# Polochon-street/bliss

Hardware: AMD Instinct MI355X
Metric: songs/sec bl_analyze (3-min 44.1kHz s16) + 10k x 10k distance-matrix sec (higher is better)
Workload: dtype f64; 1 GPU; configs[2] shard: 8192 synthetic 180-s 44.1 kHz s16 stereo songs/GPU resident (260.1 GB), 8192 total; step = analyze + all-gather + row-block distance; songs_per_gpu=8192, parallelism=shard1, fir_mode=2

## Files before the change

bliss_amd/csrc/bl_env_kernels.hip:

```cpp
#include <hip/hip_runtime.h>
#include <atomic>
#include <algorithm>
#include <stdlib.h>

#include "bl_launch.h"
#include "bl_fft_tan.h"
#include "bl_metric.h"
#include "bl_fir.h"
#include "bl_tail.h"

#define EV_CWAVES 7
#define EV_TILE (4 * EV_CWAVES)
#define EV_TROW 258

template <int CTRL> __device__ __forceinline__ double bl_dpp_f64(double v) {
  const unsigned long long b = __double_as_longlong(v);
  const int lo = __builtin_amdgcn_update_dpp(0, (int)(unsigned)(b & 0xFFFFFFFFull), CTRL, 0xF, 0xF, true);
  const int hi = __builtin_amdgcn_update_dpp(0, (int)(unsigned)(b >> 32), CTRL, 0xF, 0xF, true);
  return __longlong_as_double(((unsigned long long)(unsigned)hi << 32) | (unsigned)lo);
}

template <int CTRL> __device__ __forceinline__ double bl_dpp_f64_old(double old, double v) {
  const unsigned long long b = __double_as_longlong(v), o = __double_as_longlong(old);
  const int lo = __builtin_amdgcn_update_dpp((int)(unsigned)(o & 0xFFFFFFFFull), (int)(unsigned)(b & 0xFFFFFFFFull),
// ... 69 lines not shown
  const int n_units = EV_CWAVES * (int)gridDim.x;
  auto run_begin = [&](int u) -> int { return (int)((long long)n_rounds * u / n_units); };
  const int u0 = EV_CWAVES * (int)blockIdx.x;
  int steps = 0;
  for (int c = 0; c < EV_CWAVES; ++c) steps = max(steps, run_begin(u0 + c + 1) - run_begin(u0 + c));
  const int n_used = 256 * (sg.n_windows + 1);
  int seq = 0;

  if (wave == EV_CWAVES) {
    __builtin_amdgcn_s_setprio(3);
    {
      const int rowi = min(ln & 31, EV_TILE - 1);
      const bool own = ln < 32;
      const int c2 = min(rowi >> 2, EV_CWAVES - 1);
      const int q0 = run_begin(u0 + c2), q1 = run_begin(u0 + c2 + 1);
      const double2 *row = reinterpret_cast<const double2 *>(terms + rowi * EV_TROW);
      const double2 *zero2 = reinterpret_cast<const double2 *>(smem + EV3_ZERO_OFF);
      const double2 *tp = own ? row : row + 65;
      const double2 *tail = own ? row + 64 : zero2;
      float psum = 0.f;
      for (int st = 1; st <= steps + 1; ++st) {
        stamp(st - 1, 0);
        for (;;) {
          const int f = ln < EV_CWAVES ? flags[ln] : st;
          if (__all(f >= st)) break;
          __builtin_amdgcn_s_sleep(1);
        }
        ev_lds_acquire();
        stamp(st - 1, 1);
        const int rr = own ? st : st - 1;
        const int rho = q0 + rr - 1, w = 4 * rho + (ln & 3);
        const bool live = (ln & 31) < EV_TILE && rr >= 1 && rr <= steps && rho < q1 && w < sg.n_windows;
        const float carried = __shfl(psum, ln & 31);
        float sum = own ? 0.f : carried;
        if (live) {
          double2 ta[8], tb2[8];
#define EV_LOAD8(T, B) _Pragma("unroll") for (int k = 0; k < 8; ++k) T[k] = tp[8 * (B) + k];
#define EV_SUM8(T)                                                                                      \
  _Pragma("unroll") for (int k = 0; k < 8; ++k) {                                                       \
    sum = (float)((double)sum + T[k].x);                                                                \
    sum = (float)((double)sum + T[k].y);                                                                \
  }
#define EV_SB __builtin_amdgcn_sched_barrier(0);
          EV_LOAD8(ta, 0) EV_LOAD8(tb2, 1) EV_SB
          EV_SUM8(ta) EV_SB EV_LOAD8(ta, 2) EV_SB
          EV_SUM8(tb2) EV_SB EV_LOAD8(tb2, 3) EV_SB
          EV_SUM8(ta) EV_SB EV_LOAD8(ta, 4) EV_SB
          EV_SUM8(tb2) EV_SB EV_LOAD8(tb2, 5) EV_SB
          EV_SUM8(ta) EV_SB EV_LOAD8(ta, 6) EV_SB
          EV_SUM8(tb2) EV_SB EV_LOAD8(tb2, 7)
          const double2 tl = tail[0];
          EV_SB
          EV_SUM8(ta) EV_SB
          EV_SUM8(tb2)
          sum = (float)((double)sum + tl.x);
          sum = (float)((double)sum + tl.y);
#undef EV_LOAD8
#undef EV_SUM8
#undef EV_SB
        }
        ev_lds_release();
        if (ln == 0) flags[8] = st;
        psum = sum;
        if (live && !own) {
          energies[sg.env_off + w] = sum;
          lc[sg.env_off + w] = bl_tail_compress((double)sum, tb.log101);
        }
        stamp(st - 1, 2);
      }
    }
    return;
  }

  auto phase = [&](int k) {
    const int pr = (PRIO >> (4 * k)) & 3;
    if (pr == 0) __builtin_amdgcn_s_setprio(0);
    else if (pr == 1) __builtin_amdgcn_s_setprio(1);
    else if (pr == 2) __builtin_amdgcn_s_setprio(2);
    else __builtin_amdgcn_s_setprio(3);
  };
  double *buf = reinterpret_cast<double *>(smem) + wave * EV3_SLOTS;
  const int mean = st.mean;
  const double rcp = st.rcp, rcp_lo = st.rcp_lo;
#define FC(m) st.firc[m]
  auto nrm = [&](int k) -> double { return FIR_MODE == 2 ? (double)k : bl_norm(k, rcp, rcp_lo); };
  const int r0 = run_begin(u0 + wave), r1 = run_begin(u0 + wave + 1);
  constexpr bool EV3_TAN = FIR_MODE != 0;
  double t1[16];
  bl_fft16_fold<double> fold;
  c2d w1r[16];
  if (EV3_TAN) {
    const bl_fft_tan_lane<double> *tl = reinterpret_cast<const bl_fft_tan_lane<double> *>(tb.tan_lane) + l;
    t1[0] = 0.0;
#pragma unroll
    for (int k1 = 1; k1 < 16; ++k1) {
      t1[k1] = tl->t1[k1];
      asm volatile("" : "+v"(t1[k1]));
    }
    fold = tl->fold;
#define EV3_PIN(A, N) _Pragma("unroll") for (int i = 0; i < N; ++i) asm volatile("" : "+v"(A[i]));
    EV3_PIN(fold.rb, 4) EV3_PIN(fold.rc, 4) EV3_PIN(fold.rd, 4) EV3_PIN(fold.fb, 4) EV3_PIN(fold.fc, 2) EV3_PIN(fold.g, 3)
#undef EV3_PIN
  } else {
#pragma unroll
    for (int k1 = 1; k1 < 16; ++k1) {
      w1r[k1] = tw256[k1 * 16 + l];
      asm volatile("" : "+v"(w1r[k1].re), "+v"(w1r[k1].im));
    }
  }
  int base5 = (4 * r0) % 5;

  if (r0 < r1) {
    const int s0 = 1024 * r0 + 4 * ln;
    double r[20];
#pragma unroll
    for (int u = 0; u < 5; ++u) {
      const int i0 = s0 - 16 + 4 * u;
      const bool ok = i0 >= 0 && i0 + 4 <= n_used;
      const uint2 v = *reinterpret_cast<const uint2 *>(p + (ok ? i0 : 0));
      const unsigned w[2] = {ok ? v.x : 0u, ok ? v.y : 0u};
#pragma unroll
      for (int k = 0; k < 2; ++k) {
        const int lo = (int)(short)(w[k] & 0xFFFFu), hi = (int)(short)(w[k] >> 16);
        r[4 * u + 2 * k] = ok ? nrm(lo - mean) : 0.0;
        r[4 * u + 2 * k + 1] = ok ? nrm(hi - mean) : 0.0;
      }
    }
    double *dst = buf + base5 * EV3_BLK + EV3_ROW(ln >> 2) + EV3_UNIT(2 * (ln & 3));
#pragma unroll
    for (int i = 0; i < 4; ++i) {
#define XW(m) r[i + 16 - (m)]
      dst[EV3_UNIT(i >> 1) + (i & 1)] = BL_FIR_SEL(FIR_MODE, XW, FC);
#undef XW
    }
  }

  uint4 pre[4];
  short preh;
#if defined(__HIP_DEVICE_COMPILE__) && !defined(__gfx950__)
#error "k_env_windows3: the raw-buffer descriptor and its range check are written for gfx950"
#endif
  const __amdgpu_buffer_rsrc_t prs =
      __builtin_amdgcn_make_buffer_rsrc(const_cast<int16_t *>(p), 0, (int)(2u * (unsigned)n_used), 0x00020000);
  unsigned voff = 2u * (unsigned)(1024 * r0 + 240 + 16 * ln);
  unsigned voffh = 2u * (unsigned)(1024 * r0 + 256 * g + l);
  typedef unsigned ev_v4u __attribute__((__vector_size__(16)));
  auto fetch = [&]() {
#pragma unroll
    for (int u = 0; u < 4; ++u) {
      const ev_v4u v = __builtin_amdgcn_raw_buffer_load_b128(prs, (int)(voff + 16u * u), 0, 0);
      pre[u] = make_uint4(v[0], v[1], v[2], v[3]);
    }
    preh = (short)__builtin_amdgcn_raw_buffer_load_b16(prs, (int)voffh, 0, 0);
    voff += 2048u;
    voffh += 2048u;
  };
  fetch();
  double held[8];
#pragma unroll
  for (int k0 = 0; k0 < 8; ++k0) held[k0] = 0.0;
  auto publish_held_only = [&]() {
    while (__builtin_amdgcn_readfirstlane(flags[8]) < seq - 1) __builtin_amdgcn_s_sleep(1);
    ev_lds_acquire();
    double *tg = terms + (4 * wave + g) * EV_TROW;
#pragma unroll
    for (int k0 = 0; k0 < 8; ++k0)
      if (k0 < 7 || l != 15) tg[256 - l - 16 * k0] = held[k0];
    ev_wave_sync();
  };
  for (int s = 0; s < steps; ++s) {
    ++seq;
    const int rho = r0 + s;
    if (rho >= r1) {
      publish_held_only();
      if (ln == 0) flags[wave] = seq;
      continue;
    }
    stamp(s, 0);
    phase(0);
    double yv[16], yh;
    {
      double r[32];
#pragma unroll
      for (int u = 0; u < 4; ++u) {
        const unsigned w[4] = {pre[u].x, pre[u].y, pre[u].z, pre[u].w};
#pragma unroll
        for (int k = 0; k < 4; ++k) {
          const int lo = (int)(short)(w[k] & 0xFFFFu), hi = (int)(short)(w[k] >> 16);
          r[8 * u + 2 * k] = nrm(lo - mean);
          r[8 * u + 2 * k + 1] = nrm(hi - mean);
        }
      }
      const int kh = (int)preh - mean;
      const double xh = nrm(kh);
      fetch();
#pragma unroll
      for (int i = 0; i < 16; ++i) {
#define XR(m) r[i + 16 - (m)]
        yv[i] = BL_FIR_SEL(FIR_MODE, XR, FC);
#undef XR
      }
      if (FIR_MODE == 2) {
#define KH(m) __builtin_amdgcn_update_dpp(0, kh, 0x110 + (m), 0xF, 0xF, true)
        const double p0 = (double)kh;
        const double p1 = (double)(KH(1) + KH(15)), p2 = (double)(KH(2) + KH(14)), p3 = (double)(KH(3) + KH(13));
        const double p4 = (double)(KH(4) + KH(12)), p5 = (double)(KH(5) + KH(11)), p6 = (double)(KH(6) + KH(10));
        const double p7 = (double)(KH(7) + KH(9)), p8 = (double)KH(8);
#undef KH
        double y_ = FC(7) * p7;
        y_ = __builtin_fma(FC(6), p6, y_);
        y_ = __builtin_fma(FC(5), p5, y_);
        y_ = __builtin_fma(FC(4), p4, y_);
        y_ = __builtin_fma(FC(3), p3, y_);
        y_ = __builtin_fma(FC(2), p2, y_);
        y_ = __builtin_fma(FC(1), p1, y_);
        y_ = __builtin_fma(p8, FC(8), y_);
        yh = __builtin_fma(FC(0), p0, y_);
      } else {
      double hx[17];
      hx[0] = xh;
      hx[1] = bl_dpp_f64<0x111>(xh);  hx[2] = bl_dpp_f64<0x112>(xh);  hx[3] = bl_dpp_f64<0x113>(xh);
      hx[4] = bl_dpp_f64<0x114>(xh);  hx[5] = bl_dpp_f64<0x115>(xh);  hx[6] = bl_dpp_f64<0x116>(xh);
      hx[7] = bl_dpp_f64<0x117>(xh);  hx[8] = bl_dpp_f64<0x118>(xh);  hx[9] = bl_dpp_f64<0x119>(xh);
      hx[10] = bl_dpp_f64<0x11A>(xh); hx[11] = bl_dpp_f64<0x11B>(xh); hx[12] = bl_dpp_f64<0x11C>(xh);
      hx[13] = bl_dpp_f64<0x11D>(xh); hx[14] = bl_dpp_f64<0x11E>(xh); hx[15] = bl_dpp_f64<0x11F>(xh);
      hx[16] = 0.0;
#define XH(m) hx[m]
      yh = BL_FIR_SEL(FIR_MODE, XH, FC);
#undef XH
      }
    }
    const int xa = base5 + g, xb = xa + 1;
    const int pa = xa >= 5 ? xa - 5 : xa, pb = xb >= 5 ? xb - 5 : xb;
    double *blk_a = buf + pa * EV3_BLK, *blk_b = buf + pb * EV3_BLK;
    stamp(s, 1);
    phase(1);
    ev_wave_sync();
#pragma unroll
    for (int i = 0; i < 16; ++i) blk_b[EV3_ROW(l) + EV3_UNIT(i >> 1) + (i & 1)] = yv[i];
    buf[EV3_HEADS + ln] = yh;
    ev_wave_sync();
    double re[16], im[16];
    {
      const int off = EV3_ROW(l >> 3) + EV3_UNIT(l & 7);
      const double *ia = blk_a + off, *ib = blk_b + off;
      const double *i0 = l < 8 ? buf + EV3_HEADS + 16 * g + 2 * l : ia;
      re[0] = i0[0];
      im[0] = i0[1];
#pragma unroll
      for (int m1 = 1; m1 < 8; ++m1) { re[m1] = ia[EV3_ROW(2 * m1)]; im[m1] = ia[EV3_ROW(2 * m1) + 1]; }
#pragma unroll
      for (int m1 = 8; m1 < 16; ++m1) { re[m1] = ib[EV3_ROW(2 * (m1 - 8))]; im[m1] = ib[EV3_ROW(2 * (m1 - 8)) + 1]; }
    }
    ev_wave_sync();
    stamp(s, 2);
    phase(2);
    if (EV3_TAN) {
      bl_fft512_pass1_tan(re, im, t1);
    } else {
      bl_fft16(re, im);
#pragma unroll
      for (int k1 = 1; k1 < 16; ++k1) bl_cmul(re[bl_pos16(k1)], im[bl_pos16(k1)], w1r[k1].re, w1r[k1].im);
    }
    stamp(s, 3);
    phase(3);
    double *xg = blk_a;
    const double2 *xrow = reinterpret_cast<const double2 *>(xg + l * 18);
#pragma unroll
    for (int k1 = 0; k1 < 16; ++k1) xg[k1 * 18 + l] = re[bl_pos16(k1)];
    ev_wave_sync();
#pragma unroll
    for (int q = 0; q < 8; ++q) { const double2 v = xrow[q]; re[2 * q] = v.x; re[2 * q + 1] = v.y; }
    ev_wave_sync();
#pragma unroll
    for (int k1 = 0; k1 < 16; ++k1) xg[k1 * 18 + l] = im[bl_pos16(k1)];
    ev_wave_sync();
#pragma unroll
    for (int q = 0; q < 8; ++q) { const double2 v = xrow[q]; im[2 * q] = v.x; im[2 * q + 1] = v.y; }
    ev_wave_sync();
    stamp(s, 4);
    phase(4);
    double *tg = terms + (4 * wave + g) * EV_TROW;
    stamp(s, 5);
    phase(5);
    while (__builtin_amdgcn_readfirstlane(flags[8]) < seq - 1) {}
    ev_lds_acquire();
    stamp(s, 6);
#pragma unroll
    for (int k0 = 0; k0 < 8; ++k0)
      if (k0 < 7 || l != 15) tg[256 - l - 16 * k0] = held[k0];
    if (EV3_TAN) bl_fft16_folded(re, im, fold);
    else bl_fft16(re, im);
    double mir7 = 0.0;
#pragma unroll
    for (int k0 = 0; k0 < 8; ++k0) {
      const double sr = re[bl_pos16(15 - k0)], si = im[bl_pos16(15 - k0)];
      const double zr = k0 ? re[bl_pos16(16 - k0)] : re[bl_pos16(0)];
      const double zi = k0 ? im[bl_pos16(16 - k0)] : im[bl_pos16(0)];
      const double pr = bl_dpp_f64_old<0x111>(zr, bl_dpp_f64<0x140>(sr));
      const double pi = bl_dpp_f64_old<0x111>(zi, bl_dpp_f64<0x140>(si));
      double own;
      if (EV3_TAN)
        bl_fft512_power1_tan<double, false>(re[bl_pos16(k0)], im[bl_pos16(k0)], pr, pi, tw512[l + 16 * k0], own, held[k0]);
      else
        bl_fft512_power1<double, false>(re[bl_pos16(k0)], im[bl_pos16(k0)], pr, pi, tw512[l + 16 * k0], own, held[k0]);
      tg[l + 16 * k0] = own;
      if (k0 == 7) mir7 = held[7];
    }
    const double mr = re[bl_pos16(8)], mi = im[bl_pos16(8)];
    const double mid = 4.0 * __builtin_fma(mr, mr, mi * mi);
    if (l == 0) tg[128] = mid;
    if (l == 15) tg[129] = mir7;
    ev_wave_sync();
    if (ln == 0) flags[wave] = seq;
    stamp(s, 7);
    base5 = base5 == 0 ? 4 : base5 - 1;
  }
  ++seq;
  publish_held_only();
  if (ln == 0) flags[wave] = seq;
}
#undef FC

#define BL_TAIL_OMAX 48

__global__ __launch_bounds__(192) void k_env_tail(const bl_dsong *__restrict__ songs,
                                                  const double *__restrict__ lc, int n_songs,
                                                  bl_amd_song_result *res, int what) {
  __shared__ double yblk[2][38 * 64];
  __shared__ double oblk[2][BL_TAIL_OMAX * 64];
  __shared__ int ocnt[2][64];
  __shared__ double rings_ab[29 * 64];
  __shared__ double rings_c[19 * 64];
  __shared__ int flag_mem[4];
  typedef __attribute__((address_space(3))) volatile int lds_vint;
  lds_vint *flags = (lds_vint *)flag_mem;
  __builtin_amdgcn_s_setprio(3);
  const int wave = __builtin_amdgcn_readfirstlane(threadIdx.x >> 6), lane = threadIdx.x & 63;
  const int song = blockIdx.x * 64 + lane;
  const bool valid = song < n_songs;
  bl_dsong sg;
  if (valid) sg = songs[song];
  else { sg.nb_frames = 0; sg.n_windows = 0; sg.env_off = 0; sg.n = 1; sg.duration = 1; }
  const int N = 2 * sg.nb_frames;
  int maxN = N;
#pragma unroll
  for (int off = 32; off > 0; off >>= 1) maxN = max(maxN, __shfl_xor(maxN, off));
  if (threadIdx.x < 4) flags[threadIdx.x] = 0;
  __syncthreads();
  const int n_blocks = (maxN + 37) / 38;

  if (wave == 0) {
    bl_tail_iir a;
    a.init();
    const double *mylc = lc + sg.env_off;
    const int nw = sg.n_windows;
    auto fetch = [&](int kb_, double (&dst)[19]) {
#pragma unroll
      for (int q = 0; q < 19; ++q) dst[q] = mylc[max(min(19 * kb_ + q, nw - 1), 0)];
    };
    auto block = [&](int kb, double (&cur)[19], double (&fut)[19]) {
      if (kb >= n_blocks) return;
      fetch(kb + 2, fut);
      double *yo = yblk[kb & 1] + lane;
      double ye[38];
#pragma unroll
      for (int q = 0; q < 19; ++q) a.pair(19 * kb + q < nw ? cur[q] : 0.0, ye[2 * q], ye[2 * q + 1]);
      while (__builtin_amdgcn_readfirstlane(flags[1]) < kb - 1) __builtin_amdgcn_s_sleep(1);
      ev_lds_acquire();
#pragma unroll
      for (int q = 0; q < 38; ++q) yo[q * 64] = ye[q];
      ev_lds_release();
      bl_wave_sync();
      if (lane == 0) flags[0] = kb + 1;
    };
    double pa[19], pb[19], pc[19];
    fetch(0, pa);
    fetch(1, pb);
    for (int kb = 0; kb < n_blocks; kb += 3) {
      block(kb, pa, pc);
      block(kb + 1, pb, pa);
      block(kb + 2, pc, pb);
    }
    return;
  }

  if (wave == 1) {
    bl_tail_ab t;
    t.init(sg.nb_frames, rings_ab + lane, 64);
    for (int kb = 0; kb < n_blocks; ++kb) {
      while (__builtin_amdgcn_readfirstlane(flags[0]) < kb + 1) __builtin_amdgcn_s_sleep(1);
      while (__builtin_amdgcn_readfirstlane(flags[3]) < kb - 1) __builtin_amdgcn_s_sleep(1);
      ev_lds_acquire();
      const double *yin = yblk[kb & 1] + lane;
      const int j = 38 * kb;
      bl_tail_fifo f;
      f.base = oblk[kb & 1] + lane;
      f.stride = 64;
      f.count = 0;
      if (bl_tail_ab::chunk_ok(j, N)) {
        t.fast_chunk38(yin, 64, f.base, 64);
        f.count = 38;
      } else if (j < N) {
        for (int q = 0; q < 38; ++q) {
          const int jj = j + q;
// ... 117 lines not shown
```

bliss_amd/csrc/bl_fir.h:

```cpp
#ifndef BL_FIR_H_
#define BL_FIR_H_

#include <hip/hip_runtime.h>

#define BL_C0 (-0.0023470)
#define BL_C1 0.0044613
#define BL_C2 (-0.0114627)
#define BL_C3 0.0226382
#define BL_C4 (-0.0405147)
#define BL_C5 0.0580037
#define BL_C6 (-0.0779167)
#define BL_C7 0.0882711
#define BL_C8 0.9065095

__device__ __forceinline__ double bl_norm(int k, double rcp, double rcp_lo) {
  const double kd = (double)k;
  return __builtin_fma(kd, rcp, kd * rcp_lo);
}

#define BL_FIR(X)                                                   \
  ({                                                                \
    double y_ = BL_C7 * (X(7) + X(9));                              \
    y_ += BL_C6 * (X(6) + X(10));                                   \
    y_ += BL_C5 * (X(5) + X(11));                                   \
    y_ += BL_C4 * (X(4) + X(12));                                   \
    y_ += BL_C3 * (X(3) + X(13));                                   \
    y_ += BL_C2 * (X(2) + X(14));                                   \
    y_ += BL_C1 * (X(1) + X(15));                                   \
    y_ += X(8) * BL_C8;                                             \
    y_ += BL_C0 * (X(0) + X(16));                                   \
    y_;                                                             \
  })

#define BL_FIR_FUSED(X)                                             \
  ({                                                                \
    double y_ = BL_C7 * (X(7) + X(9));                              \
    y_ = __builtin_fma(BL_C6, X(6) + X(10), y_);                    \
    y_ = __builtin_fma(BL_C5, X(5) + X(11), y_);                    \
    y_ = __builtin_fma(BL_C4, X(4) + X(12), y_);                    \
    y_ = __builtin_fma(BL_C3, X(3) + X(13), y_);                    \
    y_ = __builtin_fma(BL_C2, X(2) + X(14), y_);                    \
    y_ = __builtin_fma(BL_C1, X(1) + X(15), y_);                    \
    y_ = __builtin_fma(X(8), BL_C8, y_);                            \
    y_ = __builtin_fma(BL_C0, X(0) + X(16), y_);                    \
    y_;                                                             \
  })
#define BL_FIR_FOLD(X, FC)                                          \
  ({                                                                \
    double y_ = FC(7) * (X(7) + X(9));                              \
    y_ = __builtin_fma(FC(6), X(6) + X(10), y_);                    \
    y_ = __builtin_fma(FC(5), X(5) + X(11), y_);                    \
    y_ = __builtin_fma(FC(4), X(4) + X(12), y_);                    \
    y_ = __builtin_fma(FC(3), X(3) + X(13), y_);                    \
    y_ = __builtin_fma(FC(2), X(2) + X(14), y_);                    \
    y_ = __builtin_fma(FC(1), X(1) + X(15), y_);                    \
    y_ = __builtin_fma(X(8), FC(8), y_);                            \
    y_ = __builtin_fma(FC(0), X(0) + X(16), y_);                    \
    y_;                                                             \
  })
#ifndef BL_FIR_FUSED_DEFAULT
#define BL_FIR_FUSED_DEFAULT 2
#endif
#define BL_FIR_SEL(MODE, X, FC) ((MODE) == 2 ? BL_FIR_FOLD(X, FC) : (MODE) == 1 ? BL_FIR_FUSED(X) : BL_FIR(X))

#endif
```

bliss_amd/csrc/bl_launch.h:

```cpp
#ifndef BL_LAUNCH_H_
#define BL_LAUNCH_H_

#include <hip/hip_runtime.h>
#include <stddef.h>
#include <stdint.h>
#include <stdio.h>

#include "bl_device.h"
#include "bl_fft.h"

#define BL_HIP_CHECK(expr)                                                              \
  do {                                                                                  \
    hipError_t e_ = (expr);                                                             \
    if (e_ != hipSuccess) {                                                             \
      fprintf(stderr, "bliss_amd: %s failed: %s (%s:%d)\n", #expr, hipGetErrorString(e_), \
              __FILE__, __LINE__);                                                      \
      return BL_UNEXPECTED;                                                             \
    }                                                                                   \
  } while (0)


struct bl_dsong {
  unsigned long long pcm_off;
  unsigned long long duration;
  long long env_off;
  int n, channels;
  int n_frames;
  int nb_frames;
  int n_windows;
  int reserved0;
  int out_idx;
  int reserved1;
};

struct bl_dstats {
  unsigned long long sum;
  unsigned long long sumsq;
  unsigned first;
  int last;
  int mean, variance;
  double vprime;
  double rcp;
  double rcp_lo;
  int wrap_pass;
  int status;
  long long wrap_acc;
  double firc[9];
};

typedef bl_c2<double> c2d;
typedef bl_c2<float> c2f;

struct bl_tables {
  const c2d *tw256_d, *tw512_d;
  const float *hann;
  const c2f *lv_tw;
  float lv_leafc[4];
  const double *tan_lane;
  const c2d *tw512t;
  double log101;
};


enum { PK_SCAN, PK_AMP, PK_FREQ, PK_FREQ_FIN, PK_ENV, PK_TAIL, PK_DIST, PK_FREQ_SCAN, PK_COUNT };

typedef void (*blk_mark_fn)(void *user, int kernel_id, hipStream_t stream, int begin);

struct Mark {
  blk_mark_fn fn;
  void *user;
  int k;
  hipStream_t s;
  Mark(blk_mark_fn f, void *u, int kk, hipStream_t ss) : fn(f), user(u), k(kk), s(ss) {
    if (fn) fn(user, k, s, 1);
  }
  ~Mark() {
    if (fn) fn(user, k, s, 0);
  }
};

inline int grid_x_for(long long units_max, int n_songs, int blocks_per_cu, int n_cu) {
  long long want = ((long long)n_cu * blocks_per_cu + n_songs - 1) / n_songs;
  if (want < 1) want = 1;
  if (want > units_max) want = units_max;
  if (want < 1) want = 1;
  if (want > 65535) want = 65535;
  return (int)want;
}


size_t blk_tables_bytes(void);
void blk_tables_fill_host(unsigned char *h);
bl_tables blk_tables_bind(const void *d_mem);
int blk_configure_device(void);

struct blk_analyze_args {
  const int16_t *pcm;
  const bl_dsong *songs;
  bl_dstats *stats;
  unsigned *hist;
  float *spectrum;
  float *energies;
  double *lc;
  bl_amd_song_result *results;
  int n_songs, max_n, what, n_cu;
  int n_head = 0, max_n_rest = 0;
  bl_tables tb;
  hipStream_t stream, side;
  hipEvent_t ev_env, ev_tail;
  hipStream_t side2 = nullptr;
  hipEvent_t ev_head = nullptr, ev_tail2 = nullptr;
  blk_mark_fn mark;
  void *mark_user;
};
int blk_analyze(const blk_analyze_args &a);


void blk_stats_init(const blk_analyze_args &a);
int blk_pcm_scan(const blk_analyze_args &a);
void blk_song_prep(const blk_analyze_args &a);
void blk_amp_finish(const blk_analyze_args &a, hipStream_t s);
void blk_force(const blk_analyze_args &a);
int blk_freq_configure_device(void);
bool blk_freq_scan_fused(int what);
void blk_freq_scan(const blk_analyze_args &a);
void blk_freq_frames(const blk_analyze_args &a, hipStream_t s);
void blk_freq_finish(const blk_analyze_args &a, hipStream_t s);
int blk_env_configure_device(void);
int blk_fir_mode();
int blk_env_windows(const blk_analyze_args &a, int fir_mode, int first, int count, int maxn);
// ... 92 lines not shown
```

bliss_amd/csrc/bl_stats_kernels.hip:

```cpp
#include <hip/hip_runtime.h>
#include <math.h>

#include "bl_launch.h"
#include "bl_scan.h"
#include "bl_fir.h"


template <bool HIST>
__global__ __launch_bounds__(256) void k_pcm_scan(const int16_t *__restrict__ pcm,
                                                  const bl_dsong *__restrict__ songs,
                                                  bl_dstats *stats, unsigned *hist) {
  __shared__ unsigned lh[BL_HIST_BINS];
  if (__builtin_amdgcn_groupstaticsize() != sizeof lh) __builtin_trap();
  const int tid = threadIdx.x;
  const bl_dsong sg = songs[blockIdx.y];
  const int16_t *p = pcm + sg.pcm_off;
  for (int i = tid; i < BL_HIST_BINS; i += 256) lh[i] = 0;
  __syncthreads();
  unsigned lds_base = (unsigned)(size_t)(bl_lds_u32 *)lh;
  asm volatile("" : "+v"(lds_base));

  long long sum = 0;
  unsigned long long sq = 0;
  const unsigned nvec = (unsigned)sg.n >> 3;
// ... 29 lines not shown
  if ((tid & 63) == 0) {
    atomicAdd(&st->sum, (unsigned long long)sum);
    atomicAdd(&st->sumsq, sq);
  }
  asm volatile("s_waitcnt lgkmcnt(0)" ::: "memory");
  __syncthreads();
  unsigned *gh = hist + (size_t)blockIdx.y * BL_HIST_BINS;
  for (int i = tid; i < BL_HIST_BINS; i += 256) {
    const unsigned c = lh[i];
    if (c) atomicAdd(&gh[i], c);
  }
}

__global__ __launch_bounds__(128) void k_trim(const int16_t *__restrict__ pcm, const bl_dsong *__restrict__ songs,
                                              bl_dstats *stats) {
  const bl_dsong sg = songs[blockIdx.x];
  const int16_t *p = pcm + sg.pcm_off;
  const uint4 *pv = reinterpret_cast<const uint4 *>(p);
  const int lane = threadIdx.x & 63, n = sg.n;
  const int nvec = n >> 3;
  const bool fwd = __builtin_amdgcn_readfirstlane(threadIdx.x >> 6) == 0;
  bl_dstats *st = stats + blockIdx.x;
  auto locate = [&](const uint4 q) -> int {
    const unsigned w[4] = {q.x, q.y, q.z, q.w};
    int at = fwd ? 8 : -1;
#pragma unroll
    for (int k = 0; k < 4; ++k) {
      if (fwd) {
        if (w[3 - k] >> 16) at = 2 * (3 - k) + 1;
        if (w[3 - k] & 0xFFFFu) at = 2 * (3 - k);
      } else {
        if (w[k] & 0xFFFFu) at = 2 * k;
        if (w[k] >> 16) at = 2 * k + 1;
      }
    }
    return at;
  };
  if (fwd) {
    unsigned first = 0xFFFFFFFFu;
    for (int v0 = 0; v0 < nvec; v0 += 128) {
      const int va = v0 + lane, vb = v0 + 64 + lane;
      const uint4 z = make_uint4(0, 0, 0, 0);
      const uint4 qa = va < nvec ? pv[va] : z, qb = vb < nvec ? pv[vb] : z;
      const unsigned long long ma = __ballot((qa.x | qa.y | qa.z | qa.w) != 0u);
      const unsigned long long mb = __ballot((qb.x | qb.y | qb.z | qb.w) != 0u);
      if (ma | mb) {
        const int src = ma ? __builtin_ctzll(ma) : __builtin_ctzll(mb);
        const unsigned mine = 8u * (unsigned)(ma ? va : vb) + (unsigned)locate(ma ? qa : qb);
        first = (unsigned)__shfl((int)mine, src);
        break;
      }
    }
    if (first == 0xFFFFFFFFu)
      for (int i = 8 * nvec; i < n; ++i)
        if (p[i] != 0) { first = (unsigned)i; break; }
    if (lane == 0) st->first = first;
  } else {
    int last = -1;
    for (int i = n - 1; i >= 8 * nvec; --i)
      if (p[i] != 0) { last = i; break; }
    if (last < 0)
      for (int v1 = nvec; v1 > 0; v1 -= 128) {
        const int va = v1 - 1 - lane, vb = v1 - 65 - lane;
        const uint4 z = make_uint4(0, 0, 0, 0);
        const uint4 qa = va >= 0 ? pv[va] : z, qb = vb >= 0 ? pv[vb] : z;
        const unsigned long long ma = __ballot((qa.x | qa.y | qa.z | qa.w) != 0u);
        const unsigned long long mb = __ballot((qb.x | qb.y | qb.z | qb.w) != 0u);
        if (ma | mb) {
          const int src = ma ? __builtin_ctzll(ma) : __builtin_ctzll(mb);
          const int mine = 8 * (ma ? va : vb) + locate(ma ? qa : qb);
          last = __shfl(mine, src);
          break;
        }
      }
    if (lane == 0) st->last = last;
  }
}

__global__ void k_stats_init(bl_dstats *stats, int n_songs) {
  const int i = blockIdx.x * blockDim.x + threadIdx.x;
  if (i >= n_songs) return;
  bl_dstats s;
  s.sum = 0; s.sumsq = 0; s.first = 0xFFFFFFFFu; s.last = -1;
  s.mean = 0; s.variance = 0; s.vprime = 0; s.rcp = 0; s.rcp_lo = 0; s.wrap_pass = 0; s.status = BL_OK;
  s.wrap_acc = 0;
  stats[i] = s;
}


__device__ __forceinline__ void prep_finish(bl_dstats &s, int n) {
  if (s.variance == 0) s.status = BL_UNEXPECTED;
  s.vprime = (double)s.variance / 32768.0;
  const double v2 = 2.0 * s.vprime;
  s.rcp = 1.0 / v2;
  s.rcp_lo = __builtin_fma(-s.rcp, v2, 1.0) / v2;
  const double taps[9] = {BL_C0, BL_C1, BL_C2, BL_C3, BL_C4, BL_C5, BL_C6, BL_C7, BL_C8};
#pragma unroll
  for (int m = 0; m < 9; ++m) s.firc[m] = __builtin_fma(taps[m], s.rcp, taps[m] * s.rcp_lo);
  (void)n;
}

__global__ void k_song_prep(const bl_dsong *__restrict__ songs, bl_dstats *stats, int n_songs,
                            bl_amd_song_result *res) {
  const int i = blockIdx.x * blockDim.x + threadIdx.x;
  if (i >= n_songs) return;
  bl_dstats s = stats[i];
  const bl_dsong sg = songs[i];
  const int n = sg.n;
  if (s.first == 0xFFFFFFFFu) {
    s.status = BL_UNEXPECTED;
    s.first = 0; s.last = n - 1;
  }
  const int wrapped = (int)(unsigned)(s.sum & 0xFFFFFFFFull);
  s.mean = wrapped / n;
  const long long m = s.mean;
  if (m > 13571 || m < -13571) {
    s.wrap_pass = 1;
  } else {
    const long long acc = (long long)s.sumsq - 2 * m * (long long)s.sum + (long long)n * m * m;
    s.variance = (int)(acc / n);
    prep_finish(s, n);
  }
  stats[i] = s;
  bl_amd_song_result *r = res + sg.out_idx;
  r->start = (int)s.first; r->end = s.last;
  r->mean = s.mean; r->variance = s.variance;
  r->n_frames = sg.n_frames; r->nb_frames = sg.nb_frames; r->n_windows = sg.n_windows;
  r->status = s.status;
}

__global__ __launch_bounds__(256) void k_variance_wrap(const int16_t *__restrict__ pcm,
                                                       const bl_dsong *__restrict__ songs,
                                                       bl_dstats *stats) {
  bl_dstats *st = stats + blockIdx.y;
  if (!st->wrap_pass) return;
  const bl_dsong sg = songs[blockIdx.y];
  const int16_t *p = pcm + sg.pcm_off;
  const int mean = st->mean;
  long long acc = 0;
  for (unsigned i = blockIdx.x * 256u + threadIdx.x; i < (unsigned)sg.n; i += gridDim.x * 256u) {
    const int v = (int)p[i] - mean;
    acc += (int)((unsigned)v * (unsigned)v);
  }
#pragma unroll
  for (int off = 32; off > 0; off >>= 1) acc += __shfl_down(acc, off);
  if ((threadIdx.x & 63) == 0)
    atomicAdd(reinterpret_cast<unsigned long long *>(&st->wrap_acc), (unsigned long long)acc);
}

__global__ void k_variance_wrap_finish(const bl_dsong *__restrict__ songs, bl_dstats *stats,
                                       int n_songs, bl_amd_song_result *res) {
  const int i = blockIdx.x * blockDim.x + threadIdx.x;
  if (i >= n_songs) return;
  bl_dstats s = stats[i];
  if (!s.wrap_pass) return;
  s.variance = (int)(s.wrap_acc / songs[i].n);
  prep_finish(s, songs[i].n);
  stats[i] = s;
  res[songs[i].out_idx].variance = s.variance;
  res[songs[i].out_idx].status = s.status;
}


#define BL_AMP_PASSES 301
#define BL_INT_LO ((32767 - 1000) - BL_HIST_LO)
#define BL_INT_HI ((32767 + 1000) - BL_HIST_LO)

__global__ __launch_bounds__(256) void k_amp_finish(const bl_dsong *__restrict__ songs,
                                                    const bl_dstats *__restrict__ stats,
                                                    const unsigned *__restrict__ hist,
                                                    bl_amd_song_result *res) {
  __shared__ float buf[2][BL_HIST_BINS + 8];
  const int tid = threadIdx.x;
  const int song = blockIdx.x;
  const bl_dstats st = stats[song];
  const int n = songs[song].n;
  const unsigned *gh = hist + (size_t)song * BL_HIST_BINS;
  const int start = (int)st.first, end = st.last;
  if (tid < 8) {
    const int c = tid < 3 ? tid : BL_HIST_BINS + tid;
    buf[0][c] = 0.f; buf[1][c] = 0.f;
// ... 111 lines not shown
```

Before: 23970 songs/s.

## Compute FIR filter with int8 MFMA on byte-split samples and integer taps

In FIR mode 2, the 17-tap symmetric FIR over raw integer PCM samples now runs on int8 matrix instructions. The integer-scaled taps are split into signed byte planes and the samples into low and high byte planes. The partial products are recombined exactly in int32 and then scaled once by a per-song factor, replacing the per-song scaled f64 tap array with a single scale. The sample fetch layout is changed to feed the MFMA operands, and the filtered outputs are scattered to the LDS ring in a new pattern. This removes many f64 FMAs per sample, at the cost of extra MFMA issue, byte permutes and a possible change in rounding from tap quantization.

```diff
diff --git a/bliss_amd/csrc/bl_env_kernels.hip b/bliss_amd/csrc/bl_env_kernels.hip
--- a/bliss_amd/csrc/bl_env_kernels.hip
+++ b/bliss_amd/csrc/bl_env_kernels.hip
@@ -175,7 +175,7 @@
   double *buf = reinterpret_cast<double *>(smem) + wave * EV3_SLOTS;
   const int mean = st.mean;
   const double rcp = st.rcp, rcp_lo = st.rcp_lo;
-#define FC(m) st.firc[m]
+  const double fsc = st.fsc;
   auto nrm = [&](int k) -> double { return FIR_MODE == 2 ? (double)k : bl_norm(k, rcp, rcp_lo); };
   const int r0 = run_begin(u0 + wave), r1 = run_begin(u0 + wave + 1);
   constexpr bool EV3_TAN = FIR_MODE != 0;
@@ -201,6 +201,19 @@
       asm volatile("" : "+v"(w1r[k1].re), "+v"(w1r[k1].im));
     }
   }
+  typedef int ev_v4i __attribute__((ext_vector_type(4)));
+  unsigned cp[4][2];
+  ev_v4i ini0, ini2, ini4;
+  if (FIR_MODE == 2) {
+    bl_firi_tap_planes(l, g, cp);
+#pragma unroll
+    for (int j = 0; j < 4; ++j) asm volatile("" : "+v"(cp[j][0]), "+v"(cp[j][1]));
+    int k0, k2, k4;
+    bl_firi_const(mean, &k0, &k2, &k4);
+    ini0 = ev_v4i{k0, k0, k0, k0};
+    ini2 = ev_v4i{k2, k2, k2, k2};
+    ini4 = ev_v4i{k4, k4, k4, k4};
+  }
   int base5 = (4 * r0) % 5;
 
   if (r0 < r1) {
@@ -223,7 +236,7 @@
 #pragma unroll
     for (int i = 0; i < 4; ++i) {
 #define XW(m) r[i + 16 - (m)]
-      dst[EV3_UNIT(i >> 1) + (i & 1)] = BL_FIR_SEL(FIR_MODE, XW, FC);
+      dst[EV3_UNIT(i >> 1) + (i & 1)] = BL_FIR_SEL(FIR_MODE, XW, fsc);
 #undef XW
     }
   }
@@ -235,13 +248,13 @@
 #endif
   const __amdgpu_buffer_rsrc_t prs =
       __builtin_amdgcn_make_buffer_rsrc(const_cast<int16_t *>(p), 0, (int)(2u * (unsigned)n_used), 0x00020000);
-  unsigned voff = 2u * (unsigned)(1024 * r0 + 240 + 16 * ln);
+  unsigned voff = 2u * (unsigned)(1024 * r0 + 240 + (FIR_MODE == 2 ? 16 * l + 8 * g : 16 * ln));
   unsigned voffh = 2u * (unsigned)(1024 * r0 + 256 * g + l);
   typedef unsigned ev_v4u __attribute__((__vector_size__(16)));
   auto fetch = [&]() {
 #pragma unroll
     for (int u = 0; u < 4; ++u) {
-      const ev_v4u v = __builtin_amdgcn_raw_buffer_load_b128(prs, (int)(voff + 16u * u), 0, 0);
+      const ev_v4u v = __builtin_amdgcn_raw_buffer_load_b128(prs, (int)(voff + (FIR_MODE == 2 ? 512u : 16u) * u), 0, 0);
       pre[u] = make_uint4(v[0], v[1], v[2], v[3]);
     }
     preh = (short)__builtin_amdgcn_raw_buffer_load_b16(prs, (int)voffh, 0, 0);
@@ -272,7 +285,42 @@
     stamp(s, 0);
     phase(0);
     double yv[16], yh;
-    {
+    const int kh = (int)preh - mean;
+    if (FIR_MODE == 2) {
+      ev_v4i acc[4][5];
+#pragma unroll
+      for (int t = 0; t < 4; ++t) {
+        const unsigned w[4] = {pre[t].x, pre[t].y, pre[t].z, pre[t].w};
+        unsigned lp[2], hp[2];
+        bl_firi_sample_planes(w, lp, hp);
+        const ev_v4i smp = {(int)lp[0], (int)lp[1], (int)hp[0], (int)hp[1]};
+        const ev_v4i zero = {0, 0, 0, 0};
+#define EV3_W64(A, B) (long)(((unsigned long long)(B) << 32) | (unsigned long long)(A))
+#define EV3_TAP2(J) ev_v4i{(int)cp[(J) + 1][0], (int)cp[(J) + 1][1], (int)cp[J][0], (int)cp[J][1]}
+        acc[t][0] = __builtin_amdgcn_mfma_i32_16x16x32_i8(EV3_W64(cp[0][0], cp[0][1]), EV3_W64(lp[0], lp[1]), ini0, 0, 0, 0);
+        acc[t][1] = __builtin_amdgcn_mfma_i32_16x16x64_i8(EV3_TAP2(0), smp, zero, 0, 0, 0);
+        acc[t][2] = __builtin_amdgcn_mfma_i32_16x16x64_i8(EV3_TAP2(1), smp, ini2, 0, 0, 0);
+        acc[t][3] = __builtin_amdgcn_mfma_i32_16x16x64_i8(EV3_TAP2(2), smp, zero, 0, 0, 0);
+        acc[t][4] = __builtin_amdgcn_mfma_i32_16x16x32_i8(EV3_W64(cp[3][0], cp[3][1]), EV3_W64(hp[0], hp[1]), ini4, 0, 0, 0);
+#undef EV3_W64
+#undef EV3_TAP2
+      }
+      fetch();
+#pragma unroll
+      for (int t = 0; t < 4; ++t)
+#pragma unroll
+        for (int r = 0; r < 4; ++r)
+          yv[4 * t + r] = bl_firi_combine(acc[t][0][r], acc[t][1][r], acc[t][2][r], acc[t][3][r], acc[t][4][r]) * fsc;
+#define KH(m) __builtin_amdgcn_update_dpp(0, kh, 0x110 + (m), 0xF, 0xF, true)
+      const double hp_[9] = {(double)kh ,
+                             (double)(KH(1) + KH(15)), (double)(KH(2) + KH(14)), (double)(KH(3) + KH(13)),
+                             (double)(KH(4) + KH(12)), (double)(KH(5) + KH(11)), (double)(KH(6) + KH(10)),
+                             (double)(KH(7) + KH(9)), (double)KH(8)};
+#undef KH
+#define XP(m) hp_[m]
+      yh = BL_FIR_INT_P(XP) * fsc;
+#undef XP
+    } else {
       double r[32];
 #pragma unroll
       for (int u = 0; u < 4; ++u) {
@@ -284,32 +332,14 @@
           r[8 * u + 2 * k + 1] = nrm(hi - mean);
         }
       }
-      const int kh = (int)preh - mean;
       const double xh = nrm(kh);
       fetch();
 #pragma unroll
       for (int i = 0; i < 16; ++i) {
 #define XR(m) r[i + 16 - (m)]
-        yv[i] = BL_FIR_SEL(FIR_MODE, XR, FC);
+        yv[i] = BL_FIR_SEL(FIR_MODE, XR, fsc);
 #undef XR
       }
-      if (FIR_MODE == 2) {
-#define KH(m) __builtin_amdgcn_update_dpp(0, kh, 0x110 + (m), 0xF, 0xF, true)
-        const double p0 = (double)kh;
-        const double p1 = (double)(KH(1) + KH(15)), p2 = (double)(KH(2) + KH(14)), p3 = (double)(KH(3) + KH(13));
-        const double p4 = (double)(KH(4) + KH(12)), p5 = (double)(KH(5) + KH(11)), p6 = (double)(KH(6) + KH(10));
-        const double p7 = (double)(KH(7) + KH(9)), p8 = (double)KH(8);
-#undef KH
-        double y_ = FC(7) * p7;
-        y_ = __builtin_fma(FC(6), p6, y_);
-        y_ = __builtin_fma(FC(5), p5, y_);
-        y_ = __builtin_fma(FC(4), p4, y_);
-        y_ = __builtin_fma(FC(3), p3, y_);
-        y_ = __builtin_fma(FC(2), p2, y_);
-        y_ = __builtin_fma(FC(1), p1, y_);
-        y_ = __builtin_fma(p8, FC(8), y_);
-        yh = __builtin_fma(FC(0), p0, y_);
-      } else {
       double hx[17];
       hx[0] = xh;
       hx[1] = bl_dpp_f64<0x111>(xh);  hx[2] = bl_dpp_f64<0x112>(xh);  hx[3] = bl_dpp_f64<0x113>(xh);
@@ -319,9 +349,8 @@
       hx[13] = bl_dpp_f64<0x11D>(xh); hx[14] = bl_dpp_f64<0x11E>(xh); hx[15] = bl_dpp_f64<0x11F>(xh);
       hx[16] = 0.0;
 #define XH(m) hx[m]
-      yh = BL_FIR_SEL(FIR_MODE, XH, FC);
+      yh = BL_FIR_SEL(FIR_MODE, XH, fsc);
 #undef XH
-      }
     }
     const int xa = base5 + g, xb = xa + 1;
     const int pa = xa >= 5 ? xa - 5 : xa, pb = xb >= 5 ? xb - 5 : xb;
@@ -329,8 +358,18 @@
     stamp(s, 1);
     phase(1);
     ev_wave_sync();
-#pragma unroll
-    for (int i = 0; i < 16; ++i) blk_b[EV3_ROW(l) + EV3_UNIT(i >> 1) + (i & 1)] = yv[i];
+    if (FIR_MODE == 2) {
+#pragma unroll
+      for (int t = 0; t < 4; ++t) {
+        const int xt = base5 + t + 1, pt = xt >= 5 ? xt - 5 : xt;
+        double *d = buf + pt * EV3_BLK + EV3_ROW(l) + EV3_UNIT(2 * g);
+#pragma unroll
+        for (int r = 0; r < 4; ++r) d[EV3_UNIT(r >> 1) + (r & 1)] = yv[4 * t + r];
+      }
+    } else {
+#pragma unroll
+      for (int i = 0; i < 16; ++i) blk_b[EV3_ROW(l) + EV3_UNIT(i >> 1) + (i & 1)] = yv[i];
+    }
     buf[EV3_HEADS + ln] = yh;
     ev_wave_sync();
     double re[16], im[16];
@@ -413,7 +452,6 @@
   publish_held_only();
   if (ln == 0) flags[wave] = seq;
 }
-#undef FC
 
 #define BL_TAIL_OMAX 48
 
diff --git a/bliss_amd/csrc/bl_fir.h b/bliss_amd/csrc/bl_fir.h
--- a/bliss_amd/csrc/bl_fir.h
+++ b/bliss_amd/csrc/bl_fir.h
@@ -2,6 +2,7 @@
 #define BL_FIR_H_
 
 #include <hip/hip_runtime.h>
+#include "bl_fir_int.h"
 
 #define BL_C0 (-0.0023470)
 #define BL_C1 0.0044613
@@ -45,22 +46,9 @@
     y_ = __builtin_fma(BL_C0, X(0) + X(16), y_);                    \
     y_;                                                             \
   })
-#define BL_FIR_FOLD(X, FC)                                          \
-  ({                                                                \
-    double y_ = FC(7) * (X(7) + X(9));                              \
-    y_ = __builtin_fma(FC(6), X(6) + X(10), y_);                    \
-    y_ = __builtin_fma(FC(5), X(5) + X(11), y_);                    \
-    y_ = __builtin_fma(FC(4), X(4) + X(12), y_);                    \
-    y_ = __builtin_fma(FC(3), X(3) + X(13), y_);                    \
-    y_ = __builtin_fma(FC(2), X(2) + X(14), y_);                    \
-    y_ = __builtin_fma(FC(1), X(1) + X(15), y_);                    \
-    y_ = __builtin_fma(X(8), FC(8), y_);                            \
-    y_ = __builtin_fma(FC(0), X(0) + X(16), y_);                    \
-    y_;                                                             \
-  })
 #ifndef BL_FIR_FUSED_DEFAULT
 #define BL_FIR_FUSED_DEFAULT 2
 #endif
-#define BL_FIR_SEL(MODE, X, FC) ((MODE) == 2 ? BL_FIR_FOLD(X, FC) : (MODE) == 1 ? BL_FIR_FUSED(X) : BL_FIR(X))
+#define BL_FIR_SEL(MODE, X, SC) ((MODE) == 2 ? BL_FIR_INT(X) * (SC) : (MODE) == 1 ? BL_FIR_FUSED(X) : BL_FIR(X))
 
 #endif
diff --git a/bliss_amd/csrc/bl_fir_int.h b/bliss_amd/csrc/bl_fir_int.h
--- /dev/null
+++ b/bliss_amd/csrc/bl_fir_int.h
@@ -0,0 +1,118 @@
+#ifndef BL_FIR_INT_H_
+#define BL_FIR_INT_H_
+
+#if defined(__HIPCC__)
+#include <hip/hip_runtime.h>
+#define BL_FIRI_HD __host__ __device__ __forceinline__
+#else
+#include <math.h>
+#define BL_FIRI_HD static inline
+#endif
+
+#define BL_CI0 (-23470.0)
+#define BL_CI1 44613.0
+#define BL_CI2 (-114627.0)
+#define BL_CI3 226382.0
+#define BL_CI4 (-405147.0)
+#define BL_CI5 580037.0
+#define BL_CI6 (-779167.0)
+#define BL_CI7 882711.0
+#define BL_CI8 9065095.0
+#define BL_FIRI_TAPSUM 9887759LL
+#define BL_FIRI_UNSCALE 1e7
+
+BL_FIRI_HD int bl_firi_tap(int m) {
+  if (m < 0 || m > 16) return 0;
+  switch (m > 8 ? 16 - m : m) {
+    case 0: return (int)BL_CI0;
+    case 1: return (int)BL_CI1;
+    case 2: return (int)BL_CI2;
+    case 3: return (int)BL_CI3;
+    case 4: return (int)BL_CI4;
+    case 5: return (int)BL_CI5;
+    case 6: return (int)BL_CI6;
+    case 7: return (int)BL_CI7;
+    default: return (int)BL_CI8;
+  }
+}
+
+BL_FIRI_HD int bl_firi_digit(int c, int j) {
+  for (int i = 0; i < j; ++i) c = (c - (int)(signed char)(c & 255)) / 256;
+  return (int)(signed char)(c & 255);
+}
+
+#define BL_FIR_INT_P(P)                                             \
+  ({                                                                \
+    double y_ = BL_CI7 * P(7);                                      \
+    y_ = __builtin_fma(BL_CI6, P(6), y_);                           \
+    y_ = __builtin_fma(BL_CI5, P(5), y_);                           \
+    y_ = __builtin_fma(BL_CI4, P(4), y_);                           \
+    y_ = __builtin_fma(BL_CI3, P(3), y_);                           \
+    y_ = __builtin_fma(BL_CI2, P(2), y_);                           \
+    y_ = __builtin_fma(BL_CI1, P(1), y_);                           \
+    y_ = __builtin_fma(P(8), BL_CI8, y_);                           \
+    y_ = __builtin_fma(BL_CI0, P(0), y_);                           \
+    y_;                                                             \
+  })
+#define BL_FIR_INT_PAIR_(X, m) ((m) == 8 ? X(8) : X(m) + X(16 - (m)))
+#define BL_FIR_INT(X)                                               \
+  ({                                                                \
+    const double ps_[9] = {BL_FIR_INT_PAIR_(X, 0), BL_FIR_INT_PAIR_(X, 1), BL_FIR_INT_PAIR_(X, 2),  \
+                           BL_FIR_INT_PAIR_(X, 3), BL_FIR_INT_PAIR_(X, 4), BL_FIR_INT_PAIR_(X, 5),  \
+                           BL_FIR_INT_PAIR_(X, 6), BL_FIR_INT_PAIR_(X, 7), BL_FIR_INT_PAIR_(X, 8)}; \
+    BL_FIR_INT_P(BL_FIR_INT_PS_);                                   \
+  })
+#define BL_FIR_INT_PS_(m) ps_[m]
+
+BL_FIRI_HD double bl_firi_scale(double rcp, double rcp_lo) {
+  const double q = rcp / BL_FIRI_UNSCALE;
+  const double r = __builtin_fma(-q, BL_FIRI_UNSCALE, rcp) + rcp_lo;
+  return q + r / BL_FIRI_UNSCALE;
+}
+
+
+BL_FIRI_HD int bl_firi_kappa(int kb, int q, int e) { return 8 * kb + 4 * q + e; }
+
+BL_FIRI_HD unsigned bl_firi_perm(unsigned hi, unsigned lo, unsigned sel) {
+#if defined(__HIP_DEVICE_COMPILE__)
+  return __builtin_amdgcn_perm(hi, lo, sel);
+#else
+  const unsigned long long v = ((unsigned long long)hi << 32) | lo;
+  unsigned r = 0;
+  for (int i = 0; i < 4; ++i) r |= (unsigned)((v >> (8 * ((sel >> (8 * i)) & 7))) & 255) << (8 * i);
+  return r;
+#endif
+}
+
+BL_FIRI_HD void bl_firi_sample_planes(const unsigned w[4], unsigned lp[2], unsigned hp[2]) {
+  for (int q = 0; q < 2; ++q) {
+    lp[q] = bl_firi_perm(w[2 * q + 1], w[2 * q], 0x06040200u) ^ 0x80808080u;
+    hp[q] = bl_firi_perm(w[2 * q + 1], w[2 * q], 0x07050301u);
+  }
+}
+
+BL_FIRI_HD void bl_firi_tap_planes(int b, int kb, unsigned cp[4][2]) {
+  for (int q = 0; q < 2; ++q) {
+    unsigned v[4] = {0, 0, 0, 0};
+    for (int e = 0; e < 4; ++e) {
+      const int c = bl_firi_tap(16 + b - bl_firi_kappa(kb, q, e));
+      for (int j = 0; j < 4; ++j) v[j] |= (unsigned)(bl_firi_digit(c, j) & 255) << (8 * e);
+    }
+    for (int j = 0; j < 4; ++j) cp[j][q] = v[j];
+  }
+}
+
+BL_FIRI_HD void bl_firi_const(int mean, int *k0, int *k2, int *k4) {
+  const long long K = (long long)(128 - mean) * BL_FIRI_TAPSUM;
+  *k0 = (int)(K & 0xFFFF);
+  *k2 = (int)((K >> 16) & 0xFFFF);
+  *k4 = (int)(K >> 32);
+}
+
+BL_FIRI_HD double bl_firi_combine(int a0, int a1, int a2, int a3, int a4) {
+  const int lo = a0 + a1 * 256;
+  const int mid = a2 + a3 * 256 + a4 * 65536;
+  return __builtin_fma((double)mid, 65536.0, (double)lo);
+}
+
+#endif
diff --git a/bliss_amd/csrc/bl_launch.h b/bliss_amd/csrc/bl_launch.h
--- a/bliss_amd/csrc/bl_launch.h
+++ b/bliss_amd/csrc/bl_launch.h
@@ -45,7 +45,7 @@
   int wrap_pass;
   int status;
   long long wrap_acc;
-  double firc[9];
+  double fsc;
 };
 
 typedef bl_c2<double> c2d;
diff --git a/bliss_amd/csrc/bl_stats_kernels.hip b/bliss_amd/csrc/bl_stats_kernels.hip
--- a/bliss_amd/csrc/bl_stats_kernels.hip
+++ b/bliss_amd/csrc/bl_stats_kernels.hip
@@ -135,7 +135,7 @@
   if (i >= n_songs) return;
   bl_dstats s;
   s.sum = 0; s.sumsq = 0; s.first = 0xFFFFFFFFu; s.last = -1;
-  s.mean = 0; s.variance = 0; s.vprime = 0; s.rcp = 0; s.rcp_lo = 0; s.wrap_pass = 0; s.status = BL_OK;
+  s.mean = 0; s.variance = 0; s.vprime = 0; s.rcp = 0; s.rcp_lo = 0; s.fsc = 0; s.wrap_pass = 0; s.status = BL_OK;
   s.wrap_acc = 0;
   stats[i] = s;
 }
@@ -147,9 +147,7 @@
   const double v2 = 2.0 * s.vprime;
   s.rcp = 1.0 / v2;
   s.rcp_lo = __builtin_fma(-s.rcp, v2, 1.0) / v2;
-  const double taps[9] = {BL_C0, BL_C1, BL_C2, BL_C3, BL_C4, BL_C5, BL_C6, BL_C7, BL_C8};
-#pragma unroll
-  for (int m = 0; m < 9; ++m) s.firc[m] = __builtin_fma(taps[m], s.rcp, taps[m] * s.rcp_lo);
+  s.fsc = bl_firi_scale(s.rcp, s.rcp_lo);
   (void)n;
 }
 
```

Measured after the change: 25860 songs/s, median of 6. 1.08x the previous value.
